# dylkot/cNMF

Hardware: AMD Instinct MI355X
Metric: NMF restarts/sec (50000x2000xK5..13) (higher is better)
Workload: dtype f32 (exact integer f16 plane x 2 f16 planes with per-row exponent, f32 accumulate)

## Files before the change

cnmf_amd/csrc/batch_host.hip.h:

```cpp
#pragma once

static int sweep_max_parts()
{
    static const int v = getenv("CNMF_SWEEP_PARTS") ? atoi(getenv("CNMF_SWEEP_PARTS")) : 64;
    return std::max(1, v);
}
static int sweep_chunks(int L) { const int64_t m = 256ll * sweep_max_parts(); return std::max(1, (int)(((int64_t)L + m - 1) / m)); }
static int sweep_parts(int L) { const int c = sweep_chunks(L); return (L + 256 * c - 1) / (256 * c); }

static int pick_nsplit(const cnmf_ctx* ctx, int KC)
{
    if (const char* s = ctx_getenv(ctx, "CNMF_NSPLIT")) { int v = atoi(s); if (v > 0) return v; }
    const int jt = (ctx->G_pad + 127) / 128;
    const int mg = std::max(1, KC / 128);
    int s = std::max(1, 512 / (jt * mg));
    const int max_by_k = std::max(1, ctx->N_pad / 256);
    return std::min(s, max_by_k);
}

static int effective_splits(int Ktot, int nsplit)
{
    const int Kper = round_up((Ktot + nsplit - 1) / nsplit, BK);
    return (Ktot + Kper - 1) / Kper;
}
// ... 212 lines not shown
        total_k += kk[r]; max_k = std::max(max_k, (int)kk[r]); min_k = std::min(min_k, (int)kk[r]);
        hoff[r + 1] = hoff[r] + (size_t)kk[r] * G;
        woff[r + 1] = woff[r] + (size_t)kk[r] * N;
    }
    const bool wide_can = gemm3_mode() != 0 && gemm3_enabled(ctx, 512);
    const char* ws_ = ctx_getenv(ctx, "CNMF_WIDE_SMALL");
    const bool wide_small = total_k >= 512 && !(ws_ && atoi(ws_) == 0);
    const bool wide_auto = wide_can && ((int64_t)ctx->N_pad * ctx->G_pad >= (1ll << 24) || wide_small);
    int KC = pick_kc(ctx, total_k, max_k, prm->kc_max, (prm->kc_max > 256 || ctx_getenv(ctx, "CNMF_KC")) ? wide_can : wide_auto);
    if (KC == 128 && prm->kc_max <= 0 && !ctx_getenv(ctx, "CNMF_KC") && gemm3_mode() >= 3 && gemm3_enabled(ctx, 256) &&
        (int64_t)ctx->N_pad * ctx->G_pad >= (1ll << 24)) {
        rc = ensure_counts(ctx);
        if (rc) return rc;
        if (ctx->count_state == 1) KC = 256;
    }
    const int KC0 = KC;
    rc = ensure_batch(ctx, KC, max_k, min_k);
    if (rc) return rc;
    rc = ensure_stage(ctx, (size_t)N * KMAX, (size_t)G * KMAX);
    if (rc) return rc;
    int nsplit = std::min(pick_nsplit(ctx, KC), ctx->nsplit_alloc);
    bool use3 = gemm3_enabled(ctx, KC);
    bool usec = false;
    if (use3 && gemm3_mode() >= 3) {
        rc = ensure_counts(ctx);
        if (rc) return rc;
        usec = ctx->count_state == 1;
    }
    static const bool g2g_off = getenv("CNMF_G2G") && atoi(getenv("CNMF_G2G")) == 0;
    bool use2g = use3 && !usec && gemm3_mode() >= 4 && !g2g_off && ctx->G_pad % G3C_JW == 0 && ctx->N_pad % G3C_JW == 0;
    if (use2g) { rc = ensure_x2planes(ctx); if (rc) return rc; }
    bool use2h = (usec && ctx->count_fmt == 4) || use2g;
    const int gemm_mode_used = !use3 ? 0 : (use2g ? 5 : (usec ? (use2h ? 4 : 3) : std::min(gemm3_mode(), 2)));
    const int KbA = ctx->G_pad / 16, KbB = ctx->N_pad / 16;
    const unsigned char *xA = use2g ? ctx->X2h : ctx->C1, *xAhi = use2g ? ctx->X2m : ctx->C1h;
    const unsigned char *xB = use2g ? ctx->Xt2h : ctx->Ct1, *xBhi = use2g ? ctx->Xt2m : ctx->Ct1h;
    const unsigned int *xAfl = use2g ? ctx->onesA : ctx->hiA, *xBfl = use2g ? ctx->onesB : ctx->hiB;
    const float *csA = use2g ? ctx->x2sA : nullptr, *csB = use2g ? ctx->x2sB : nullptr;
    const double* dsc = use2g ? nullptr : ctx->d_scale;
    const int nsubA = use2h ? gemm2h_nsub(xAhi != nullptr, KbA) : 1, nsubB = use2h ? gemm2h_nsub(xBhi != nullptr, KbB) : 1;
    static const bool fuse_off = getenv("CNMF_FUSE_W") && atoi(getenv("CNMF_FUSE_W")) == 0;
    const bool fuseW = use2h && !fuse_off && max_k <= KSMALL && ctx->shiftW != nullptr;
    int shgen = 0;
    int* const shW[2] = {ctx->shiftW, ctx->shiftW ? ctx->shiftW + ctx->kc_alloc : nullptr};
    if (fuseW) HIP_TRY(ctx, hipMemsetAsync(ctx->shiftW, 0, (size_t)3 * ctx->kc_alloc * sizeof(int), ctx->stream));
    if (use3 && !usec && !use2g) { rc = ensure_planes(ctx); if (rc) return rc; }
    const int jwA = (usec || use2g) ? G3C_JW : G3_JW;
    int nsplit3 = use3 ? pick_nsplit3(ctx, KC, jwA) : 1;
    const int nsplit3_first = nsplit3;
    const int fin_y = (max_k * max_k + 255) / 256;
    const int lag_env = ctx_getenv(ctx, "CNMF_LAG") ? atoi(ctx_getenv(ctx, "CNMF_LAG")) : 0;
    const int lag = std::max(1, std::min(RING - 2, prm->lag > 0 ? prm->lag : (lag_env > 0 ? lag_env : 2)));
    hipStream_t st = ctx->stream;

    DevPool pool;
    EventPool events;
    float* d_Hres = nullptr; float* d_Wres = nullptr;
    if (resident) {
        if (ctx->spectra_rows && ctx->spectra_G != G) {
            SET_ERR(ctx, "the resident store holds spectra over %lld genes, this matrix has %d: cnmf_spectra_reset first",
                    (long long)ctx->spectra_G, G);
            return CNMF_ESTATE;
        }
        ctx->spectra_G = G;
        const size_t need = (ctx->spectra_rows + (size_t)total_k) * G;
        if (need > ctx->spectra_cap) {
            float* nb = nullptr;
            const size_t cap = std::max(need, ctx->spectra_cap * 2);
            HIP_TRY(ctx, hipMalloc(&nb, cap * sizeof(float)));
            hipError_t ce = hipSuccess;
            if (ctx->spectra_rows)
                ce = hipMemcpyAsync(nb, ctx->spectra, ctx->spectra_rows * G * sizeof(float), hipMemcpyDeviceToDevice, st);
            if (ce == hipSuccess) ce = hipStreamSynchronize(st);
            if (ce != hipSuccess) { hipFree(nb); HIP_TRY(ctx, ce); }
            hipFree(ctx->spectra);
            ctx->spectra = nb; ctx->spectra_cap = cap;
        }
        d_Hres = ctx->spectra + ctx->spectra_rows * G;
    } else {
        d_Hres = pool.get<float>(hoff[n]);
    }
    if (W_out) d_Wres = pool.get<float>(woff[n]);
    int* d_repack = pool.get<int>((size_t)3 * KC0);
    POOL_TRY(ctx, pool);
    struct PinnedInts { int* p = nullptr; ~PinnedInts() { if (p) hipHostFree(p); } } repack_host;
    HIP_TRY(ctx, hipHostMalloc(&repack_host.p, (size_t)RING * 3 * KC0 * sizeof(int)));
    int* h_repack = repack_host.p;

    float *d_H0 = nullptr, *d_Wt0 = nullptr;
    RngJob* d_jobs = nullptr;
    if (init_mode == 1) {
        d_H0 = pool.get<float>(hoff[n]);
        d_Wt0 = pool.get<float>(woff[n]);
        d_jobs = pool.get<RngJob>((size_t)n);
        POOL_TRY(ctx, pool);
        std::vector<RngJob> jobs(n);
        int rowoff = 0;
        for (int r = 0; r < n; ++r) {
            jobs[r] = RngJob{seeds[r], kk[r], rowoff, avg[r], (long long)kk[r] * ((long long)G + N)};
            rowoff += kk[r];
        }
        HIP_TRY(ctx, hipMemcpy(d_jobs, jobs.data(), (size_t)n * sizeof(RngJob), hipMemcpyHostToDevice));
        rng_kernel<1><<<n, 256, 0, st>>>(d_jobs, nullptr, d_H0, G, G, d_Wt0, N, N);
        HIP_TRY(ctx, hipGetLastError());
    }

    std::vector<int> order(n);
    const bool queue_by_rank = ctx_getenv(ctx, "CNMF_QUEUE") && !strcmp(ctx_getenv(ctx, "CNMF_QUEUE"), "rank");
    const bool have_prior = ctx->iter_hint.size() == (size_t)KMAX + 1;
    auto prior_of = [&](int k) { return have_prior ? ctx->iter_hint[k] : 0.0; };
    if (queue_by_rank) {
        for (int r = 0; r < n; ++r) order[r] = r;
        std::stable_sort(order.begin(), order.end(), [&](int a, int b) { return kk[a] > kk[b]; });
    } else {
        std::vector<std::vector<int>> by_k(KMAX + 1);
        for (int r = 0; r < n; ++r) by_k[kk[r]].push_back(r);
        size_t pos = 0;
        for (size_t j = 0; pos < (size_t)n; ++j)
            for (int k = KMAX; k >= 1; --k)
                if (j < by_k[k].size()) order[pos++] = by_k[k][j];
        if (have_prior)
            std::stable_sort(order.begin(), order.end(), [&](int a, int b) {
                const double ea = prior_of(kk[a]) > 0 ? prior_of(kk[a]) : 1e30, eb = prior_of(kk[b]) > 0 ? prior_of(kk[b]) : 1e30;
                return ea > eb;
            });
    }
    std::vector<int64_t> k_iters(KMAX + 1, 0), k_done(KMAX + 1, 0);
    std::vector<double> rank_expect(KMAX + 1, 1e30);
    static const bool holes_fill = !(getenv("CNMF_HOLES") && !strcmp(getenv("CNMF_HOLES"), "wait"));
    if (have_prior)
        for (int k = 1; k <= KMAX; ++k) if (prior_of(k) > 0) rank_expect[k] = prior_of(k);
    int last_resort_done = 0;
    size_t next = 0;
    int n_pending = n;

    ColAlloc cols(KC);
    std::vector<HostSlot> hs(KC0);
    int nslots = 0;
    int n_active = 0;
    int64_t it = 0;
    int snap_nslots[RING] = {0};
    const bool no_defrag = ctx_getenv(ctx, "CNMF_NO_DEFRAG") != nullptr;
    const bool no_psum = ctx_getenv(ctx, "CNMF_NO_PSUM") != nullptr;
    const bool no_part = ctx_getenv(ctx, "CNMF_PART") == nullptr || ctx_getenv(ctx, "CNMF_NO_PART") != nullptr;
    int64_t last_tail_repack = -1000;
    int64_t last_defrag = -8, n_defrag = 0;
    bool h3_valid = false;
    memset(ctx->h_snap, 0, (size_t)ctx->kc_alloc * RING * sizeof(SlotDesc));
    hipEvent_t ev_begin = events.get(), ev_end = events.get();
    POOL_TRY(ctx, events);
    HIP_TRY(ctx, hipEventRecord(ev_begin, st));
    const int time_stride = !stats ? 0 : (prm->profile > 0 ? prm->profile : (ctx_getenv(ctx, "CNMF_TIME_GEMM") ? 1 : 0));
    std::vector<hipEvent_t> gev;

    const int chunksW = sweep_chunks(N), partsW = sweep_parts(N);
    const int chunksH = sweep_chunks(G), partsH = sweep_parts(G);
    const float l1W = (float)prm->l1_reg_W, l2W = (float)prm->l2_reg_W;
    const float l1H = (float)prm->l1_reg_H, l2H = (float)prm->l2_reg_H;
    const int gvarA = ctx_getenv(ctx, "CNMF_GEMM_A") ? atoi(ctx_getenv(ctx, "CNMF_GEMM_A")) : 0;
    const int gvarB = ctx_getenv(ctx, "CNMF_GEMM_B") ? atoi(ctx_getenv(ctx, "CNMF_GEMM_B")) : 0;
    int64_t restart_iters = 0, column_iters = 0, restart_col_iters = 0;
    const bool dbg = ctx_getenv(ctx, "CNMF_DEBUG") != nullptr;
    int64_t dbg_it[65] = {0}, dbg_live[65] = {0};
    const int wg_slots = ctx_getenv(ctx, "CNMF_SK_WGS") ? atoi(ctx_getenv(ctx, "CNMF_SK_WGS")) : 2 * 256;
    StreamK sk = plan_streamk(KC, ctx->N_pad, ctx->G_pad, wg_slots);
    if (sk.on) HIP_TRY(ctx, hipMemcpyAsync(ctx->d_split, sk.split.data(), sk.split.size(), hipMemcpyHostToDevice, st));
    int nsplitA = (sk.on && gvarA == 0) ? 1 : std::min(pick_nsplit_A(ctx, KC), ctx->nsplitA_alloc);
    StreamK3 sk3;
    if (use3) {
        sk3 = plan_streamk3(KC, ctx->N_pad, ctx->G_pad, gemm3_wg_slots(), jwA, nsubA);
        if (sk3.on) HIP_TRY(ctx, hipMemcpyAsync(ctx->d_split, sk3.flags.data(), sk3.flags.size(), hipMemcpyHostToDevice, st));
        else nsplitA = std::min(pick_nsplit_A3(ctx, KC, jwA), ctx->nsplitA_alloc);
    }
    int n_done = 0;
    hipEvent_t ev_tail = nullptr;
    int64_t tail_its = 0, tail_live = 0;

    auto retire = [&](int s, const SlotDesc& snap) -> int {
        HostSlot& h = hs[s];
        const int r = h.restart, k = h.k;
        dim3 gH((G + 255) / 256, k), gW((N + 255) / 256, k);
        extract_kernel<<<gH, 256, 0, st>>>(ctx->H, ctx->G_pad, G, h.off, k, d_Hres + hoff[r], 0);
        if (d_Wres) extract_kernel<<<gW, 256, 0, st>>>(ctx->Wt, ctx->N_pad, N, h.off, k, d_Wres + woff[r], 1);
        clear_rows_kernel<<<gH, 256, 0, st>>>(ctx->H, ctx->G_pad, ctx->G_pad, h.off, k);
        clear_rows_kernel<<<gW, 256, 0, st>>>(ctx->Wt, ctx->N_pad, ctx->N_pad, h.off, k);
        HIP_TRY(ctx, hipGetLastError());
        if (n_iter_out) n_iter_out[r] = snap.iter;
        if (viol_out) viol_out[r] = snap.viol_last;
        restart_iters += snap.iter;
        restart_col_iters += (int64_t)snap.iter * k;
        k_iters[k] += snap.iter; k_done[k] += 1;
        if (n_pending > 0) cols.release(h.off, k);
        h.state = 0; h.restart = -1;
        --n_active; ++n_done;
        return CNMF_OK;
    };

    int n_repack = 0;
    auto repack_left = [&](int width, bool balanced = false) -> int {
        std::vector<int> idx;
        for (int s = 0; s < nslots; ++s) if (hs[s].state) idx.push_back(s);
        std::sort(idx.begin(), idx.end(), [&](int a, int b) { return hs[a].off < hs[b].off; });
        int* hm = h_repack + (size_t)(n_repack++ % RING) * 3 * KC0;
        int* d_colmap = d_repack, *d_ids = d_repack + KC0, *d_offs = d_repack + 2 * KC0;
        int pos = 0, nmove = 0;
        const int ngroups = width / 256;
        if (balanced && ngroups > 1) {
            for (int c = 0; c < width; ++c) hm[c] = -1;
            std::vector<int> fill(ngroups, 0), byk(idx);
            std::stable_sort(byk.begin(), byk.end(), [&](int a, int b) { return hs[a].k > hs[b].k; });
            bool ok = true;
            std::vector<int> newoff(nslots, -1);
            for (int s : byk) {
                int g = -1;
                for (int q = 0; q < ngroups; ++q) if (fill[q] + hs[s].k <= 256 && (g < 0 || fill[q] < fill[g])) g = q;
                if (g < 0) { ok = false; break; }
                newoff[s] = g * 256 + fill[g]; fill[g] += hs[s].k;
            }
            if (ok) {
                for (int s : idx) {
                    HostSlot& h = hs[s];
                    for (int c = 0; c < h.k; ++c) hm[newoff[s] + c] = h.off + c;
                    if (h.off != newoff[s]) { hm[KC0 + nmove] = s; hm[2 * KC0 + nmove] = newoff[s]; ++nmove; h.off = newoff[s]; }
                }
                pos = 0;
            } else balanced = false;
        } else balanced = false;
        if (!balanced) {
        for (int s : idx) {
            HostSlot& h = hs[s];
            for (int c = 0; c < h.k; ++c) hm[pos + c] = h.off + c;
            if (h.off != pos) { hm[KC0 + nmove] = s; hm[2 * KC0 + nmove] = pos; ++nmove; h.off = pos; }
            pos += h.k;
        }
        for (int c = pos; c < width; ++c) hm[c] = -1;
        }
        if (nmove || pos < width) {
            HIP_TRY(ctx, hipMemcpyAsync(d_colmap, hm, (size_t)width * sizeof(int), hipMemcpyHostToDevice, st));
            gather_rows_cm_kernel<<<dim3((ctx->N_pad / 4 + 255) / 256, width), 256, 0, st>>>(ctx->Wt, ctx->N_pad, d_colmap, ctx->XHt);
            gather_rows_cm_kernel<<<dim3((ctx->G_pad / 4 + 255) / 256, width), 256, 0, st>>>(ctx->H, ctx->G_pad, d_colmap, ctx->XtW);
            HIP_TRY(ctx, hipGetLastError());
            HIP_TRY(ctx, hipMemcpyAsync(ctx->Wt, ctx->XHt, (size_t)width * ctx->N_pad * sizeof(float), hipMemcpyDeviceToDevice, st));
            HIP_TRY(ctx, hipMemcpyAsync(ctx->H, ctx->XtW, (size_t)width * ctx->G_pad * sizeof(float), hipMemcpyDeviceToDevice, st));
            if (fuseW) {
                int* tmp = ctx->shiftW + 2 * ctx->kc_alloc;
                for (int g2 = 0; g2 < 2; ++g2) {
                    permute_ints_kernel<<<(width + 255) / 256, 256, 0, st>>>(shW[g2], d_colmap, tmp, width);
                    HIP_TRY(ctx, hipMemcpyAsync(shW[g2], tmp, (size_t)width * sizeof(int), hipMemcpyDeviceToDevice, st));
                }
                HIP_TRY(ctx, hipGetLastError());
            }
            if (nmove) {
                HIP_TRY(ctx, hipMemcpyAsync(d_ids, hm + KC0, (size_t)nmove * sizeof(int), hipMemcpyHostToDevice, st));
                HIP_TRY(ctx, hipMemcpyAsync(d_offs, hm + 2 * KC0, (size_t)nmove * sizeof(int), hipMemcpyHostToDevice, st));
                set_slot_offs_kernel<<<(nmove + 255) / 256, 256, 0, st>>>(ctx->d_slots, d_ids, d_offs, nmove);
                HIP_TRY(ctx, hipGetLastError());
            }
        }
        h3_valid = false;
        if (use2h) HIP_TRY(ctx, launch_rowmax_part(st, ctx->Wt, ctx->N_pad, N, KC, chunksW * 256, nullptr, partsW, ctx->rmaxW));
        return CNMF_OK;
    };

    auto refill = [&](int& n_new) -> int {
        n_new = 0;
        int* new_list = ctx->h_slot_list + (size_t)(it % RING) * KC0;
        for (int attempt = 0; attempt < 2; ++attempt) {
        int failed_k = 1 << 30;
        int head_k = 0; double head_expect = 0.0;
        for (size_t pi = next; pi < order.size() && n_pending > 0; ++pi) {
            const int r = order[pi];
            if (r < 0) { if (pi == next) ++next; continue; }
            const int k = kk[r];
            if (k >= failed_k) continue;
            if (head_k && !holes_fill && !(rank_expect[k] < 0.3 * head_expect)) continue;
            const int off = cols.alloc(k);
            if (off < 0) {
                failed_k = k;
                if (!head_k) { head_k = k; head_expect = rank_expect[k]; }
                continue;
            }
            order[pi] = -1; --n_pending;
            if (pi == next) ++next;
            int s = 0;
            while (s < KC0 && hs[s].state != 0) ++s;
            hs[s].state = 1; hs[s].restart = r; hs[s].off = off; hs[s].k = k; hs[s].installed_at = it;
            nslots = std::max(nslots, s + 1);
            dim3 gI((std::max(N, G) + 255) / 256, k);
            if (init_mode == 0) {
                HIP_TRY(ctx, hipMemcpyAsync(ctx->stageH, H0 + hoff[r], (size_t)k * G * sizeof(float), hipMemcpyHostToDevice, st));
                HIP_TRY(ctx, hipMemcpyAsync(ctx->stageW, W0 + woff[r], (size_t)k * N * sizeof(float), hipMemcpyHostToDevice, st));
                install_kernel<<<gI, 256, 0, st>>>(ctx->stageH, ctx->stageW, ctx->H, ctx->G_pad, G, ctx->Wt, ctx->N_pad, N, off, k);
            } else {
                install_cm_kernel<<<gI, 256, 0, st>>>(d_H0 + hoff[r], d_Wt0 + woff[r], ctx->H, ctx->G_pad, G, ctx->Wt, ctx->N_pad, N, off);
            }
            HIP_TRY(ctx, hipGetLastError());
            if (fuseW) {
                float mx = 0.f;
                if (init_mode == 1) mx = 6.0f * (float)avg[r];
                else for (size_t q = 0; q < (size_t)k * N; ++q) mx = std::max(mx, W0[woff[r] + q]);
                int e2 = 0;
                if (mx > 0.f) std::frexp(mx, &e2);
                const int sh0 = mx > 0.f ? std::max(-110, std::min(120, 13 - e2)) : 0;
                set_ints_kernel<<<1, 128, 0, st>>>(shW[0], shW[1], off, k, sh0);
                HIP_TRY(ctx, hipGetLastError());
            }
            SlotDesc* d = &ctx->h_slots[s];
            memset(d, 0, sizeof *d);
            d->off = off; d->k = k; d->active = 1; d->iter = 0; d->restart = r;
            HIP_TRY(ctx, hipMemcpyAsync(ctx->d_slots + s, d, sizeof(SlotDesc), hipMemcpyHostToDevice, st));
            new_list[n_new++] = s;
            ++n_active;
        }
        if (attempt == 0 && n_pending > 0 && failed_k < (1 << 30) && !no_defrag && it - last_defrag >= 8) {
            int live_cols = 0;
            for (int s2 = 0; s2 < nslots; ++s2) if (hs[s2].state) live_cols += hs[s2].k;
            if (KC - live_cols >= (holes_fill ? failed_k : head_k)) {
                int rcd = repack_left(KC);
                if (rcd) return rcd;
                cols = ColAlloc(KC);
                for (int s2 = 0; s2 < nslots; ++s2) if (hs[s2].state) cols.alloc(hs[s2].k);
                last_defrag = it; ++n_defrag;
                continue;
            }
        }
        break;
        }
        if (n_new) {
            int* dl = ctx->d_slot_list + (size_t)(it % RING) * KC0;
            HIP_TRY(ctx, hipMemcpyAsync(dl, new_list, n_new * sizeof(int), hipMemcpyHostToDevice, st));
            gram_rows_kernel<<<n_new, 256, 0, st>>>(ctx->H, ctx->G_pad, G, ctx->d_slots, dl, ctx->gramH, l2W);
            HIP_TRY(ctx, hipGetLastError());
        }
        return CNMF_OK;
    };

    auto iterate = [&](int n_new) -> int {
        int tiers = 0;
        for (int s2 = 0; s2 < nslots; ++s2)
            if (hs[s2].state) tiers |= hs[s2].k <= 16 ? 1 : (hs[s2].k <= 32 ? 2 : (hs[s2].k <= KSMALL ? 4 : 8));
        unsigned long long livemask = ~0ull;
        if (use2h && n_pending == 0 && !no_part) {
            livemask = 0ull;
            for (int s2 = 0; s2 < nslots; ++s2)
                if (hs[s2].state)
                    for (int t = hs[s2].off / 32; t <= (hs[s2].off + hs[s2].k - 1) / 32 && t < 64; ++t) livemask |= 1ull << t;
            int fullest = 0;
            for (int g = 0; g < KC / 256; ++g) fullest = std::max(fullest, __builtin_popcountll((livemask >> (8 * g)) & 0xffull));
            if (fullest > 6) livemask = ~0ull;
        }
        const bool time_gemm = time_stride > 0 && it % time_stride == 0;
        if (time_gemm) {
            for (int i = 0; i < 4; ++i) gev.push_back(events.get());
            POOL_TRY(ctx, events);
            hipEventRecord(gev[gev.size() - 4], st);
        }
        SplitInfo spA{nullptr, nullptr, 1, 1, 1};
        if (use3) {
            if ((n_new > 0 || !h3_valid) && use2h) {
                HIP_TRY(ctx, launch_rowmax_part(st, ctx->H, ctx->G_pad, G, KC, chunksH * 256, dsc, partsH, ctx->rmaxH));
                HIP_TRY(ctx, launch_split2h(st, ctx->H, ctx->G_pad, KC, ctx->G_pad, ctx->H3, G3_MW, dsc, ctx->rmaxH,
                                            partsH, ctx->iscaleH));
            } else if (n_new > 0 || !h3_valid)
                HIP_TRY(ctx, launch_split3(st, ctx->H, ctx->G_pad, KC, ctx->G_pad, ctx->H3, G3_MW, usec ? ctx->d_scale : nullptr));
            if (time_gemm) hipEventRecord(gev[gev.size() - 4], st);
            if (sk3.on) {
                if (use2h) {
                    HIP_TRY(ctx, launch_gemm2h_streamk(st, sk3, ctx->H3, xA, xAhi, xAfl, ctx->iscaleH, KbA,
                                                       ctx->XHt, ctx->XHt1, ctx->XHt2, ctx->N_pad, csA, livemask));
                }
                else if (usec)
                    HIP_TRY(ctx, launch_gemm3c_streamk(st, sk3, ctx->H3, ctx->C1, ctx->C1h, ctx->hiA, ctx->XHt, ctx->XHt1,
                                                       ctx->XHt2, ctx->N_pad));
                else
                    HIP_TRY(ctx, launch_gemm3_streamk(st, sk3, ctx->H3, ctx->X3, ctx->XHt, ctx->XHt1, ctx->XHt2, ctx->N_pad));
                spA = SplitInfo{ctx->XHt1, ctx->d_split, jwA, G3_MW, sk3.MG, ctx->XHt2};
            } else if (use2h) {
                HIP_TRY(ctx, launch_gemm2h(st, ctx->H3, xA, xAhi, xAfl, ctx->iscaleH, KbA, ctx->XHt, ctx->N_pad,
                                           (long long)KC * ctx->N_pad, KC, ctx->N_pad, nsplitA, csA, livemask));
            } else if (usec) {
                HIP_TRY(ctx, launch_gemm3c(st, ctx->H3, ctx->C1, ctx->C1h, ctx->hiA, ctx->G_pad / 16, ctx->XHt, ctx->N_pad,
                                           (long long)KC * ctx->N_pad, KC, ctx->N_pad, nsplitA));
            } else {
                HIP_TRY(ctx, launch_gemm3(st, ctx->H3, ctx->X3, ctx->G_pad / 16, ctx->XHt, ctx->N_pad,
                                          (long long)KC * ctx->N_pad, KC, ctx->N_pad, nsplitA));
            }
        } else if (sk.on && gvarA == 0) {
            HIP_TRY(ctx, launch_streamk_passA(st, sk, ctx->H, ctx->G_pad, ctx->X, ctx->G_pad, ctx->XHt,
                                              ctx->XHt1, ctx->N_pad, ctx->N_pad));
            spA = SplitInfo{ctx->XHt1, ctx->d_split, 128, sk.mw, sk.MG};
        } else
            HIP_TRY(ctx, launch_gemm<false>(st, gvarA, ctx->H, ctx->G_pad, ctx->X, ctx->G_pad, ctx->XHt,
                                            ctx->N_pad, (long long)KC * ctx->N_pad, KC, ctx->G_pad, ctx->N_pad, nsplitA));
        if (time_gemm) hipEventRecord(gev[gev.size() - 3], st);
        if (!spA.plane1)
            HIP_TRY(ctx, launch_reduce_splits(st, ctx->XHt, use2h ? gemm2h_splits(KbA, nsplitA, nsubA) : nsplitA,
                                              (long long)KC * ctx->N_pad, (long long)KC * ctx->N_pad));
        const bool fuse_now = fuseW && use2h;
        HIP_TRY(ctx, launch_sweep(st, nslots, ctx->Wt, ctx->N_pad, N, ctx->XHt, ctx->gramH,
                                  ctx->d_slots, l1W, ctx->gram_part, ctx->viol_part, chunksW, partsW, 1, max_k, tiers, spA,
                                  use2h ? ctx->rmaxW : nullptr, nullptr, false,
                                  fuse_now ? PlaneOut{(unsigned short*)ctx->Wt3, shW[shgen], KbB, G3_MW} : PlaneOut{nullptr, nullptr, 0, 0}));
        if (use2h) {
            const FinalizeArgs fa{ctx->gram_part, ctx->viol_part, partsW, ctx->gramW, l2H, ctx->d_slots, 0, prm->tol,
                                  prm->max_iter, 1, max_k, nullptr, 0};
            HIP_TRY(ctx, launch_split2h_finalize(st, ctx->Wt, ctx->N_pad, KC, ctx->N_pad, ctx->Wt3, G3_MW, nullptr, ctx->rmaxW,
                                                 partsW, ctx->iscaleW, fa, nslots, fin_y,
                                                 fuse_now ? SplitFused{shW[shgen], shW[shgen ^ 1]} : SplitFused{nullptr, nullptr}));
            if (fuse_now) shgen ^= 1;
        } else if (use3) {
            const FinalizeArgs fa{ctx->gram_part, ctx->viol_part, partsW, ctx->gramW, l2H, ctx->d_slots, 0, prm->tol,
                                  prm->max_iter, 1, max_k, nullptr, 0};
            HIP_TRY(ctx, launch_split3_finalize(st, ctx->Wt, ctx->N_pad, KC, ctx->N_pad, ctx->Wt3, G3_MW, nullptr, fa,
                                                nslots, fin_y));
        } else {
            finalize_kernel<<<dim3(nslots, fin_y), 256, 0, st>>>(ctx->gram_part, ctx->viol_part, partsW, ctx->gramW, l2H,
                                                    ctx->d_slots, 0, prm->tol, prm->max_iter, 1, max_k);
        }
        if (time_gemm) hipEventRecord(gev[gev.size() - 2], st);
        const int nsB = use2h ? gemm2h_splits(KbB, nsplit3, nsubB) : (use3 ? nsplit3 : nsplit);
        if (use2h)
            HIP_TRY(ctx, launch_gemm2h(st, ctx->Wt3, xB, xBhi, xBfl, ctx->iscaleW, KbB, ctx->XtW, ctx->G_pad,
                                       (long long)KC * ctx->G_pad, KC, ctx->G_pad, nsplit3, csB, livemask));
        else if (usec)
            HIP_TRY(ctx, launch_gemm3c(st, ctx->Wt3, ctx->Ct1, ctx->Ct1h, ctx->hiB, ctx->N_pad / 16, ctx->XtW, ctx->G_pad,
                                       (long long)KC * ctx->G_pad, KC, ctx->G_pad, nsplit3));
        else if (use3)
            HIP_TRY(ctx, launch_gemm3(st, ctx->Wt3, ctx->Xt3, ctx->N_pad / 16, ctx->XtW, ctx->G_pad,
                                      (long long)KC * ctx->G_pad, KC, ctx->G_pad, nsplit3));
        else
            HIP_TRY(ctx, launch_gemm<true>(st, gvarB, ctx->Wt, ctx->N_pad, ctx->X, ctx->G_pad, ctx->XtW,
                                           ctx->G_pad, (long long)KC * ctx->G_pad, KC, ctx->N_pad,
                                           ctx->G_pad, nsplit));
        if (time_gemm) hipEventRecord(gev[gev.size() - 1], st);
        if (use2h && !no_psum && !(tiers & 8)) {
            HIP_TRY(ctx, launch_sweep(st, nslots, ctx->H, ctx->G_pad, G, ctx->XtW, ctx->gramW,
                                      ctx->d_slots, l1H, ctx->gram_part, ctx->viol_part, chunksH, partsH, 1, max_k, tiers,
                                      psum_info(nsB, (long long)KC * ctx->G_pad, dsc), ctx->rmaxH, dsc, true));
        } else {
            HIP_TRY(ctx, launch_reduce_splits(st, ctx->XtW, nsB, (long long)KC * ctx->G_pad,
                                              (long long)KC * ctx->G_pad, usec ? dsc : nullptr, ctx->G_pad));
            HIP_TRY(ctx, launch_sweep(st, nslots, ctx->H, ctx->G_pad, G, ctx->XtW, ctx->gramW,
                                      ctx->d_slots, l1H, ctx->gram_part, ctx->viol_part, chunksH, partsH, 1, max_k, tiers,
                                      SplitInfo{nullptr, nullptr, 1, 1, 1}, use2h ? ctx->rmaxH : nullptr,
                                      use2h ? dsc : nullptr));
        }
        SlotDesc* snap = ctx->h_snap + (size_t)(it % RING) * KC0;
        SlotDesc* snap_dev = nullptr;
        HIP_TRY(ctx, hipHostGetDevicePointer((void**)&snap_dev, snap, 0));
        if (use2h) {
            const FinalizeArgs fa{ctx->gram_part, ctx->viol_part, partsH, ctx->gramH, l2W, ctx->d_slots, 1, prm->tol,
                                  prm->max_iter, 1, max_k, snap_dev, (int)(it + 1)};
            HIP_TRY(ctx, launch_split2h_finalize(st, ctx->H, ctx->G_pad, KC, ctx->G_pad, ctx->H3, G3_MW, dsc,
                                                 ctx->rmaxH, partsH, ctx->iscaleH, fa, nslots, fin_y));
            h3_valid = true;
        } else if (use3) {
            const FinalizeArgs fa{ctx->gram_part, ctx->viol_part, partsH, ctx->gramH, l2W, ctx->d_slots, 1, prm->tol,
                                  prm->max_iter, 1, max_k, snap_dev, (int)(it + 1)};
            HIP_TRY(ctx, launch_split3_finalize(st, ctx->H, ctx->G_pad, KC, ctx->G_pad, ctx->H3, G3_MW,
                                                usec ? ctx->d_scale : nullptr, fa, nslots, fin_y));
            h3_valid = true;
        } else {
            finalize_kernel<<<dim3(nslots, fin_y), 256, 0, st>>>(ctx->gram_part, ctx->viol_part, partsH, ctx->gramH, l2W,
                                                    ctx->d_slots, 1, prm->tol, prm->max_iter, 1, max_k,
                                                    snap_dev, (int)(it + 1));
        }
        HIP_TRY(ctx, hipGetLastError());
        snap_nslots[it % RING] = nslots;
        column_iters += KC;
        if (n_pending == 0) {
            int live = 0;
            for (int s2 = 0; s2 < nslots; ++s2) if (hs[s2].state) live += hs[s2].k;
            ++tail_its; tail_live += live;
        }
        if (dbg) {
            int live = 0;
            for (int s2 = 0; s2 < nslots; ++s2) if (hs[s2].state) live += hs[s2].k;
            dbg_it[KC / 32] += 1; dbg_live[KC / 32] += live;
        }
        ++it;
        return CNMF_OK;
    };

    auto inspect = [&]() -> int {
        const int64_t si = it - 1 - lag;
        if (si < 0) return CNMF_OK;
        const SlotDesc* sp = ctx->h_snap + (size_t)(si % RING) * KC0;
        int rc2 = wait_snapshot(ctx, sp, snap_nslots[si % RING], (int)(si + 1));
        if (rc2) return rc2;
        for (int s = 0; s < snap_nslots[si % RING]; ++s)
            if (hs[s].state == 1 && hs[s].installed_at <= si && sp[s].active == 0 && sp[s].restart == hs[s].restart) {
                rc2 = retire(s, sp[s]);
                if (rc2) return rc2;
            }
        if (!queue_by_rank && n_pending > 1 && n_done - last_resort_done >= 8) {
            last_resort_done = n_done;
            std::vector<int> rest;
            rest.reserve(n_pending);
            for (size_t pi = next; pi < order.size(); ++pi) if (order[pi] >= 0) rest.push_back(order[pi]);
            std::vector<double> fly_age(KMAX + 1, 0.0); std::vector<int> fly_n(KMAX + 1, 0);
            for (int s2 = 0; s2 < nslots; ++s2)
                if (hs[s2].state) { fly_age[hs[s2].k] += (double)(it - hs[s2].installed_at); fly_n[hs[s2].k] += 1; }
            auto expect = [&](int r) {
                const int k = kk[r];
                double num = (double)k_iters[k] + fly_age[k], den = (double)k_done[k] + fly_n[k];
                if (prior_of(k) > 0) { num += 4.0 * prior_of(k); den += 4.0; }
                return den > 0 ? num / den : 1e30;
            };
            for (int k = 1; k <= KMAX; ++k) {
                const double den = (double)k_done[k] + fly_n[k] + (prior_of(k) > 0 ? 4.0 : 0.0);
                if (den > 0) rank_expect[k] = ((double)k_iters[k] + fly_age[k] + 4.0 * prior_of(k)) / den;
            }
            if (dbg && n_done % 64 < 8) {
                fprintf(stderr, "[cnmf] it %lld done %d pending %d expected per rank:", (long long)it, n_done, n_pending);
                for (int k = 1; k <= KMAX; ++k)
                    if (k_done[k] + fly_n[k] > 0)
                        fprintf(stderr, " k%d=%.0f(%lld done, %d fly)", k, ((double)k_iters[k] + fly_age[k]) / ((double)k_done[k] + fly_n[k]),
                                (long long)k_done[k], fly_n[k]);
                fprintf(stderr, "\n");
            }
            std::stable_sort(rest.begin(), rest.end(), [&](int a, int b) {
                const double ea = expect(a), eb = expect(b);
                return ea != eb ? ea > eb : kk[a] > kk[b];
            });
            order.resize(next);
            order.insert(order.end(), rest.begin(), rest.end());
        }
        return CNMF_OK;
    };

    const bool no_compact = ctx_getenv(ctx, "CNMF_NO_COMPACT") != nullptr;
    const bool f32_tail = ctx_getenv(ctx, "CNMF_F32_TAIL") != nullptr;
    auto compact = [&]() -> int {
        if (n_pending == 0 && n_active > 0 && KC > 32 && !no_compact) {
            int live_cols = 0;
            for (int s = 0; s < nslots; ++s) if (hs[s].state) live_cols += hs[s].k;
            int KCn = 32;
            while (KCn < live_cols && KCn < 256) KCn *= 2;
            if (live_cols > 256) KCn = round_up(live_cols, 256);
            bool stay3 = false;
            if (use3 && !f32_tail && KCn > (usec ? 32 : 64)) { KCn = round_up(std::max(live_cols, 1), 256); stay3 = true; }
            if (KCn == KC && use2h && !no_part && it - last_tail_repack >= 16) {
                unsigned long long m = 0ull;
                for (int s = 0; s < nslots; ++s)
                    if (hs[s].state)
                        for (int t = hs[s].off / 32; t <= (hs[s].off + hs[s].k - 1) / 32 && t < 64; ++t) m |= 1ull << t;
                const int ng = KC / 256;
                int fullest = 0;
                for (int g = 0; g < ng; ++g) fullest = std::max(fullest, __builtin_popcountll((m >> (8 * g)) & 0xffull));
                const int ideal = ((live_cols + 31) / 32 + ng - 1) / ng;
                if (ideal <= 6 && fullest >= ideal + 2) {
                    int rcp = repack_left(KC, true);
                    if (rcp) return rcp;
                    last_tail_repack = it;
                }
            }
            if (KCn < KC) {
                last_tail_repack = it;
                int rcp = repack_left(KCn, stay3 && use2h && !no_part);
                if (rcp) return rcp;
                KC = KCn;
                cols = ColAlloc(KC);
                for (int s = 0; s < nslots; ++s) if (hs[s].state) cols.alloc(hs[s].k);
                const int cap = (ctx->nsplit_alloc * KC0) / KC;
                if (stay3) {
                    nsplit3 = std::max(1, std::min(pick_nsplit3(ctx, KC, jwA), cap));
                    sk3 = plan_streamk3(KC, ctx->N_pad, ctx->G_pad, gemm3_wg_slots(), jwA, nsubA);
                    if (sk3.on) HIP_TRY(ctx, hipMemcpyAsync(ctx->d_split, sk3.flags.data(), sk3.flags.size(), hipMemcpyHostToDevice, st));
                    else nsplitA = std::max(1, std::min(pick_nsplit_A3(ctx, KC, jwA), (ctx->nsplitA_alloc * KC0) / KC));
                } else {
                nsplit = std::max(1, std::min(pick_nsplit(ctx, KC), cap));
                use3 = usec = use2h = use2g = false;
                sk = plan_streamk(KC, ctx->N_pad, ctx->G_pad, wg_slots);
                nsplitA = (sk.on && gvarA == 0) ? 1
                        : std::max(1, std::min(pick_nsplit_A(ctx, KC), (ctx->nsplitA_alloc * KC0) / KC));
                if (sk.on) {
                    HIP_TRY(ctx, hipMemcpyAsync(ctx->d_split, sk.split.data(), sk.split.size(), hipMemcpyHostToDevice, st));
// ... 167 lines not shown
```

cnmf_amd/csrc/cnmf_hip.hip:

```cpp
#include <hip/hip_runtime.h>

#include <algorithm>
#include <chrono>
#include <cmath>
#include <cstdint>
#include <cstdio>
#include <cstdlib>
#include <cstring>
#include <functional>
#include <string>
#include <vector>

#include "../../include/cnmf_hip.h"
#ifdef CNMF_DEBUG_ABI
#include "../../include/cnmf_hip_debug.h"
#endif
#include "kernels_gemm.hip.h"
#include "kernels_gemm3.hip.h"
#include "kernels_counts.hip.h"
#include "kernels_gemm2h.hip.h"
#include "kernels_rng.hip.h"
#include "kernels_sweep.hip.h"

using namespace cnmf;

#include "runtime.hip.h"
#include "csr_host.hip.h"
#include "gemm_host.hip.h"

extern "C" int cnmf_device_count(void)
{
    int n = 0;
    if (hipGetDeviceCount(&n) != hipSuccess) return 0;
    return n;
}

extern "C" const char* cnmf_version(void) { return "cnmf_hip 0.1.0 (gfx950)"; }

extern "C" const char* cnmf_last_error(const cnmf_ctx* ctx)
{
    return ctx ? ctx->err.c_str() : g_last_error.c_str();
}

extern "C" cnmf_ctx* cnmf_create(int device)
{
    int n = 0;
    hipError_t e = hipGetDeviceCount(&n);
    if (e != hipSuccess || n <= 0) {
        SET_ERR((cnmf_ctx*)nullptr, "no HIP device available (%s)", hipGetErrorString(e));
        return nullptr;
    }
    if (device < 0 || device >= n) {
        SET_ERR((cnmf_ctx*)nullptr, "device %d out of range (have %d)", device, n);
        return nullptr;
    }
    if (hipSetDevice(device) != hipSuccess) {
        SET_ERR((cnmf_ctx*)nullptr, "hipSetDevice(%d) failed", device);
        return nullptr;
    }
    cnmf_ctx* ctx = new cnmf_ctx();
    ctx_snapshot_env(ctx);
    ctx->device = device;
    if (hipStreamCreateWithFlags(&ctx->stream, hipStreamNonBlocking) != hipSuccess) {
        SET_ERR((cnmf_ctx*)nullptr, "hipStreamCreate failed");
        delete ctx;
        return nullptr;
    }
    return ctx;
}

extern "C" int cnmf_reload_env(cnmf_ctx* ctx)
{
    if (!ctx) return CNMF_EINVAL;
    ctx_snapshot_env(ctx);
    return CNMF_OK;
}

static void free_x2(cnmf_ctx* c)
{
    hipFree(c->X2h); hipFree(c->X2m); hipFree(c->Xt2h); hipFree(c->Xt2m); hipFree(c->x2sA); hipFree(c->x2sB);
    hipFree(c->onesA); hipFree(c->onesB);
    c->X2h = c->X2m = c->Xt2h = c->Xt2m = nullptr; c->x2sA = c->x2sB = nullptr; c->onesA = c->onesB = nullptr;
}

static void free_mu_sparse(cnmf_ctx* c)
{
    for (int i = 0; i < 2; ++i) { c->spA[i].release(); c->spB[i].release(); }
    c->x_nnz = -1;
}

static void free_batch(cnmf_ctx* c)
{
    hipFree(c->H); hipFree(c->Wt); hipFree(c->XHt); hipFree(c->XHt1); hipFree(c->XHt2); hipFree(c->XtW); hipFree(c->d_split);
    hipFree(c->H3); hipFree(c->Wt3);
    hipFree(c->rmaxH); hipFree(c->rmaxW); hipFree(c->iscaleH); hipFree(c->iscaleW); hipFree(c->shiftW);
    c->rmaxH = c->rmaxW = c->iscaleH = c->iscaleW = nullptr; c->shiftW = nullptr;
    c->XHt1 = c->XHt2 = nullptr; c->d_split = nullptr; c->H3 = c->Wt3 = nullptr;
    hipFree(c->gramH); hipFree(c->gramW); hipFree(c->gram_part); hipFree(c->viol_part);
    hipFree(c->d_slots); hipFree(c->d_slot_list);
    if (c->h_slots) hipHostFree(c->h_slots);
    if (c->h_snap) hipHostFree(c->h_snap);
    if (c->h_slot_list) hipHostFree(c->h_slot_list);
    c->H = c->Wt = c->XHt = c->XtW = c->gramH = c->gramW = c->gram_part = nullptr;
    c->viol_part = nullptr; c->d_slots = nullptr; c->d_slot_list = nullptr;
    c->h_slots = c->h_snap = nullptr; c->h_slot_list = nullptr;
// ... 192 lines not shown
```

Before: 221.6.

## Batch slot install and retire into event tables with fused kernels

Replaces the per-restart sequence of extract, clear, install, set_ints, SlotDesc memcpy and gram_rows launches with batched event tables. Each table is uploaded in one memcpy and processed by one fused retire kernel, or by an install kernel plus a gram-finish kernel. The Gram matrix of the initial H is now computed from the source buffer as chunked partials reduced in double. This cuts launch and small-copy overhead per restart. In exchange it adds pinned and device event buffers and a gram partial workspace, whose capacity limit forces extra flushes.

```diff
diff --git a/cnmf_amd/csrc/batch_host.hip.h b/cnmf_amd/csrc/batch_host.hip.h
--- a/cnmf_amd/csrc/batch_host.hip.h
+++ b/cnmf_amd/csrc/batch_host.hip.h
@@ -318,10 +318,19 @@
     }
     if (W_out) d_Wres = pool.get<float>(woff[n]);
     int* d_repack = pool.get<int>((size_t)3 * KC0);
+    const size_t evt_region = (size_t)KC0 * (sizeof(SlotRow) + sizeof(int) + 8);
+    unsigned char* d_evt = pool.get<unsigned char>(evt_region);
+    const int gram0_gc = max_k <= KSMALL ? 128 : 64;
+    const size_t gram0_per_slot = (size_t)((G + gram0_gc - 1) / gram0_gc) * max_k * max_k;
+    const int gram0_cap = (int)std::max<size_t>(1, std::min<size_t>((size_t)KC0 / min_k + 1, ((size_t)8 << 20) / gram0_per_slot));
+    float* d_gram0 = pool.get<float>((size_t)gram0_cap * gram0_per_slot);
     POOL_TRY(ctx, pool);
     struct PinnedInts { int* p = nullptr; ~PinnedInts() { if (p) hipHostFree(p); } } repack_host;
     HIP_TRY(ctx, hipHostMalloc(&repack_host.p, (size_t)RING * 3 * KC0 * sizeof(int)));
     int* h_repack = repack_host.p;
+    struct PinnedBytes { unsigned char* p = nullptr; ~PinnedBytes() { if (p) hipHostFree(p); } } evt_host;
+    HIP_TRY(ctx, hipHostMalloc(&evt_host.p, (size_t)RING * 2 * evt_region));
+    unsigned char* h_evt = evt_host.p;
 
     float *d_H0 = nullptr, *d_Wt0 = nullptr;
     RngJob* d_jobs = nullptr;
@@ -412,15 +421,68 @@
     hipEvent_t ev_tail = nullptr;
     int64_t tail_its = 0, tail_live = 0;
 
+    struct SlotEvent {
+        int64_t epoch = -1;
+        size_t used = 0;
+        SlotRow* rows = nullptr;
+        int nrows = 0, max_k = 0, stage_rows = 0;
+        std::vector<int> heads;
+    } ev_ret, ev_ins;
+    auto event_add = [&](SlotEvent& e, int kind, int s, long long hpos, long long wpos, int sh0) -> int {
+        const HostSlot& h = hs[s];
+        if (e.nrows == 0) {
+            if (e.epoch != it) { e.epoch = it; e.used = 0; }
+            e.rows = reinterpret_cast<SlotRow*>(h_evt + ((size_t)(it % RING) * 2 + kind) * evt_region + e.used);
+            e.max_k = 0; e.heads.clear();
+        }
+        if (e.used + (size_t)(e.nrows + h.k) * sizeof(SlotRow) + (e.heads.size() + 1) * sizeof(int) > evt_region) {
+            SET_ERR(ctx, "slot event table overflow (%d rows)", e.nrows + h.k);
+            return CNMF_ESTATE;
+        }
+        e.heads.push_back(e.nrows);
+        for (int c = 0; c < h.k; ++c) e.rows[e.nrows++] = SlotRow{h.off + c, h.k, c, s, hpos, wpos, sh0, h.restart, {0, 0}};
+        e.max_k = std::max(e.max_k, h.k);
+        return CNMF_OK;
+    };
+    auto event_upload = [&](SlotEvent& e) -> int {
+        memcpy(e.rows + e.nrows, e.heads.data(), e.heads.size() * sizeof(int));
+        const size_t bytes = (size_t)e.nrows * sizeof(SlotRow) + e.heads.size() * sizeof(int);
+        HIP_TRY(ctx, hipMemcpyAsync(d_evt, e.rows, bytes, hipMemcpyHostToDevice, st));
+        e.used += (bytes + 7) & ~(size_t)7;
+        return CNMF_OK;
+    };
+    auto flush_retire = [&]() -> int {
+        if (ev_ret.nrows == 0) return CNMF_OK;
+        if (int rcu = event_upload(ev_ret)) return rcu;
+        dim3 grid((std::max(ctx->G_pad, ctx->N_pad) + SLOT_CHUNK - 1) / SLOT_CHUNK, ev_ret.nrows);
+        slots_retire_kernel<<<grid, 256, 0, st>>>(reinterpret_cast<const SlotRow*>(d_evt), ctx->H, ctx->G_pad, G,
+                                                 ctx->Wt, ctx->N_pad, N, d_Hres, d_Wres);
+        HIP_TRY(ctx, hipGetLastError());
+        ev_ret.nrows = 0;
+        return CNMF_OK;
+    };
+    auto flush_install = [&]() -> int {
+        if (ev_ins.nrows == 0) return CNMF_OK;
+        if (int rcu = event_upload(ev_ins)) return rcu;
+        const SlotRow* d_rows = reinterpret_cast<const SlotRow*>(d_evt);
+        const int* d_heads = reinterpret_cast<const int*>(d_rows + ev_ins.nrows);
+        const int nsl = (int)ev_ins.heads.size(), gc = ev_ins.max_k <= KSMALL ? 128 : 64;
+        const int nch = (G + gc - 1) / gc, kk = ev_ins.max_k * ev_ins.max_k;
+        const int xch = (std::max(N, G) + SLOT_CHUNK - 1) / SLOT_CHUNK;
+        slots_install_kernel<<<xch * ev_ins.nrows + nch * nsl, 256, 0, st>>>(
+            d_rows, d_heads, ev_ins.nrows, xch, init_mode == 0 ? ctx->stageH : d_H0, init_mode == 0 ? ctx->stageW : d_Wt0,
+            init_mode == 0 ? 1 : 0, ctx->H, ctx->G_pad, G, ctx->Wt, ctx->N_pad, N, fuseW ? shW[0] : nullptr,
+            fuseW ? shW[1] : nullptr, ctx->d_slots, d_gram0, nch, kk);
+        slots_gram_finish_kernel<<<nsl, 256, 0, st>>>(d_rows, d_heads, d_gram0, nch, kk, G, ctx->gramH, l2W);
+        HIP_TRY(ctx, hipGetLastError());
+        ev_ins.nrows = 0; ev_ins.stage_rows = 0;
+        return CNMF_OK;
+    };
+
     auto retire = [&](int s, const SlotDesc& snap) -> int {
         HostSlot& h = hs[s];
         const int r = h.restart, k = h.k;
-        dim3 gH((G + 255) / 256, k), gW((N + 255) / 256, k);
-        extract_kernel<<<gH, 256, 0, st>>>(ctx->H, ctx->G_pad, G, h.off, k, d_Hres + hoff[r], 0);
-        if (d_Wres) extract_kernel<<<gW, 256, 0, st>>>(ctx->Wt, ctx->N_pad, N, h.off, k, d_Wres + woff[r], 1);
-        clear_rows_kernel<<<gH, 256, 0, st>>>(ctx->H, ctx->G_pad, ctx->G_pad, h.off, k);
-        clear_rows_kernel<<<gW, 256, 0, st>>>(ctx->Wt, ctx->N_pad, ctx->N_pad, h.off, k);
-        HIP_TRY(ctx, hipGetLastError());
+        if (int rce = event_add(ev_ret, 0, s, (long long)hoff[r], (long long)woff[r], 0)) return rce;
         if (n_iter_out) n_iter_out[r] = snap.iter;
         if (viol_out) viol_out[r] = snap.viol_last;
         restart_iters += snap.iter;
@@ -500,7 +562,6 @@
 
     auto refill = [&](int& n_new) -> int {
         n_new = 0;
-        int* new_list = ctx->h_slot_list + (size_t)(it % RING) * KC0;
         for (int attempt = 0; attempt < 2; ++attempt) {
         int failed_k = 1 << 30;
         int head_k = 0; double head_expect = 0.0;
@@ -522,36 +583,33 @@
             while (s < KC0 && hs[s].state != 0) ++s;
             hs[s].state = 1; hs[s].restart = r; hs[s].off = off; hs[s].k = k; hs[s].installed_at = it;
             nslots = std::max(nslots, s + 1);
-            dim3 gI((std::max(N, G) + 255) / 256, k);
+            if (ev_ins.nrows && ((int)ev_ins.heads.size() >= gram0_cap || (init_mode == 0 && ev_ins.stage_rows + k > KMAX)))
+                if (int rcf = flush_install()) return rcf;
+            long long hpos = (long long)hoff[r], wpos = (long long)woff[r];
             if (init_mode == 0) {
-                HIP_TRY(ctx, hipMemcpyAsync(ctx->stageH, H0 + hoff[r], (size_t)k * G * sizeof(float), hipMemcpyHostToDevice, st));
-                HIP_TRY(ctx, hipMemcpyAsync(ctx->stageW, W0 + woff[r], (size_t)k * N * sizeof(float), hipMemcpyHostToDevice, st));
-                install_kernel<<<gI, 256, 0, st>>>(ctx->stageH, ctx->stageW, ctx->H, ctx->G_pad, G, ctx->Wt, ctx->N_pad, N, off, k);
-            } else {
-                install_cm_kernel<<<gI, 256, 0, st>>>(d_H0 + hoff[r], d_Wt0 + woff[r], ctx->H, ctx->G_pad, G, ctx->Wt, ctx->N_pad, N, off);
-            }
-            HIP_TRY(ctx, hipGetLastError());
+                hpos = (long long)ev_ins.stage_rows * G; wpos = (long long)ev_ins.stage_rows * N;
+                HIP_TRY(ctx, hipMemcpyAsync(ctx->stageH + hpos, H0 + hoff[r], (size_t)k * G * sizeof(float), hipMemcpyHostToDevice, st));
+                HIP_TRY(ctx, hipMemcpyAsync(ctx->stageW + wpos, W0 + woff[r], (size_t)k * N * sizeof(float), hipMemcpyHostToDevice, st));
+                ev_ins.stage_rows += k;
+            }
+            int sh0 = 0;
             if (fuseW) {
                 float mx = 0.f;
                 if (init_mode == 1) mx = 6.0f * (float)avg[r];
                 else for (size_t q = 0; q < (size_t)k * N; ++q) mx = std::max(mx, W0[woff[r] + q]);
                 int e2 = 0;
                 if (mx > 0.f) std::frexp(mx, &e2);
-                const int sh0 = mx > 0.f ? std::max(-110, std::min(120, 13 - e2)) : 0;
-                set_ints_kernel<<<1, 128, 0, st>>>(shW[0], shW[1], off, k, sh0);
-                HIP_TRY(ctx, hipGetLastError());
-            }
-            SlotDesc* d = &ctx->h_slots[s];
-            memset(d, 0, sizeof *d);
-            d->off = off; d->k = k; d->active = 1; d->iter = 0; d->restart = r;
-            HIP_TRY(ctx, hipMemcpyAsync(ctx->d_slots + s, d, sizeof(SlotDesc), hipMemcpyHostToDevice, st));
-            new_list[n_new++] = s;
+                sh0 = mx > 0.f ? std::max(-110, std::min(120, 13 - e2)) : 0;
+            }
+            if (int rce = event_add(ev_ins, 1, s, hpos, wpos, sh0)) return rce;
+            ++n_new;
             ++n_active;
         }
         if (attempt == 0 && n_pending > 0 && failed_k < (1 << 30) && !no_defrag && it - last_defrag >= 8) {
             int live_cols = 0;
             for (int s2 = 0; s2 < nslots; ++s2) if (hs[s2].state) live_cols += hs[s2].k;
             if (KC - live_cols >= (holes_fill ? failed_k : head_k)) {
+                if (int rcf = flush_install()) return rcf;
                 int rcd = repack_left(KC);
                 if (rcd) return rcd;
                 cols = ColAlloc(KC);
@@ -562,13 +620,7 @@
         }
         break;
         }
-        if (n_new) {
-            int* dl = ctx->d_slot_list + (size_t)(it % RING) * KC0;
-            HIP_TRY(ctx, hipMemcpyAsync(dl, new_list, n_new * sizeof(int), hipMemcpyHostToDevice, st));
-            gram_rows_kernel<<<n_new, 256, 0, st>>>(ctx->H, ctx->G_pad, G, ctx->d_slots, dl, ctx->gramH, l2W);
-            HIP_TRY(ctx, hipGetLastError());
-        }
-        return CNMF_OK;
+        return flush_install();
     };
 
     auto iterate = [&](int n_new) -> int {
@@ -729,6 +781,7 @@
                 rc2 = retire(s, sp[s]);
                 if (rc2) return rc2;
             }
+        if ((rc2 = flush_retire())) return rc2;
         if (!queue_by_rank && n_pending > 1 && n_done - last_resort_done >= 8) {
             last_resort_done = n_done;
             std::vector<int> rest;
diff --git a/cnmf_amd/csrc/cnmf_hip.hip b/cnmf_amd/csrc/cnmf_hip.hip
--- a/cnmf_amd/csrc/cnmf_hip.hip
+++ b/cnmf_amd/csrc/cnmf_hip.hip
@@ -21,6 +21,7 @@
 #include "kernels_gemm2h.hip.h"
 #include "kernels_rng.hip.h"
 #include "kernels_sweep.hip.h"
+#include "kernels_slots.hip.h"
 
 using namespace cnmf;
 
diff --git a/cnmf_amd/csrc/kernels_slots.hip.h b/cnmf_amd/csrc/kernels_slots.hip.h
--- /dev/null
+++ b/cnmf_amd/csrc/kernels_slots.hip.h
@@ -0,0 +1,133 @@
+#pragma once
+#include <hip/hip_runtime.h>
+#include "kernels_sweep.hip.h"
+
+namespace cnmf {
+
+struct SlotRow {
+    int row;
+    int k;
+    int c;
+    int slot;
+    long long hpos;
+    long long wpos;
+    int sh0;
+    int restart;
+    int pad_[2];
+};
+static_assert(sizeof(SlotRow) == 48, "SlotRow is copied as raw bytes");
+
+constexpr int SLOT_CHUNK = 1024;
+
+__global__ __launch_bounds__(256) void slots_retire_kernel(const SlotRow* __restrict__ rows,
+                                                           float* __restrict__ H, int ldh, int G,
+                                                           float* __restrict__ Wt, int ldw, int N,
+                                                           float* __restrict__ Hres, float* __restrict__ Wres)
+{
+    const SlotRow r = rows[blockIdx.y];
+    float* h = H + (size_t)r.row * ldh;
+    float* w = Wt + (size_t)r.row * ldw;
+    float* ho = Hres + r.hpos + (size_t)r.c * G;
+    float* wo = Wres ? Wres + r.wpos + r.c : nullptr;
+#pragma unroll
+    for (int j = 0; j < SLOT_CHUNK / 256; ++j) {
+        const int i = blockIdx.x * SLOT_CHUNK + j * 256 + threadIdx.x;
+        if (i < ldh) {
+            if (i < G) ho[i] = h[i];
+            h[i] = 0.f;
+        }
+        if (i < ldw) {
+            if (wo && i < N) wo[(size_t)i * r.k] = w[i];
+            w[i] = 0.f;
+        }
+    }
+}
+
+template <int GC>
+__device__ __forceinline__ void gram_chunk_body(const float* __restrict__ src, int ld, int L, int k, int g0,
+                                                float* __restrict__ part, float* lds)
+{
+    float (*tile)[GC + 1] = reinterpret_cast<float (*)[GC + 1]>(lds);
+    const int tid = threadIdx.x;
+    for (int e = tid; e < k * GC; e += 256) {
+        const int c = e / GC, g = e % GC;
+        tile[c][g] = (g0 + g < L) ? src[(size_t)c * ld + g0 + g] : 0.f;
+    }
+    __syncthreads();
+    for (int e = tid; e < k * k; e += 256) {
+        const int a = e / k, b = e % k;
+        float s = 0.f;
+        for (int g = 0; g < GC; ++g) s = fmaf(tile[a][g], tile[b][g], s);
+        part[e] = s;
+    }
+}
+
+__global__ __launch_bounds__(256) void slots_install_kernel(const SlotRow* __restrict__ rows, const int* __restrict__ heads,
+                                                            int nrows, int xch,
+                                                            const float* __restrict__ H0, const float* __restrict__ W0, int w_rowmajor,
+                                                            float* __restrict__ H, int ldh, int G,
+                                                            float* __restrict__ Wt, int ldw, int N,
+                                                            int* __restrict__ shA, int* __restrict__ shB,
+                                                            SlotDesc* __restrict__ slots,
+                                                            float* __restrict__ gram_part, int nch, int kk)
+{
+    __shared__ __attribute__((aligned(16))) float lds[KMAX * 65];
+    const int b = blockIdx.x;
+    if (b < xch * nrows) {
+        const SlotRow r = rows[b / xch];
+        const int xc = b % xch;
+        const float* hs = H0 + r.hpos + (size_t)r.c * G;
+        const float* ws = w_rowmajor ? W0 + r.wpos + r.c : W0 + r.wpos + (size_t)r.c * N;
+        const size_t wstep = w_rowmajor ? (size_t)r.k : 1;
+        float* h = H + (size_t)r.row * ldh;
+        float* w = Wt + (size_t)r.row * ldw;
+#pragma unroll
+        for (int j = 0; j < SLOT_CHUNK / 256; ++j) {
+            const int i = xc * SLOT_CHUNK + j * 256 + threadIdx.x;
+            if (i < G) h[i] = hs[i];
+            if (i < N) w[i] = ws[(size_t)i * wstep];
+        }
+        if (xc == 0 && threadIdx.x == 0) {
+            if (shA) { shA[r.row] = r.sh0; shB[r.row] = r.sh0; }
+            if (r.c == 0) {
+                SlotDesc d;
+                d.off = r.row; d.k = r.k; d.active = 1; d.iter = 0; d.restart = r.restart; d.pad_ = 0;
+                d.viol = 0.0; d.viol_init = 0.0; d.viol_last = 0.0;
+                slots[r.slot] = d;
+            }
+        }
+    } else {
+        const int gb = b - xch * nrows;
+        const int j = gb / nch, chunk = gb % nch;
+        const SlotRow r = rows[heads[j]];
+        const float* src = H0 + r.hpos;
+        float* part = gram_part + ((size_t)j * nch + chunk) * kk;
+        if (r.k <= KSMALL) {
+            if (chunk * 128 < G) gram_chunk_body<128>(src, G, G, r.k, chunk * 128, part, lds);
+        } else {
+            if (chunk * 64 < G) gram_chunk_body<64>(src, G, G, r.k, chunk * 64, part, lds);
+        }
+    }
+}
+
+__global__ __launch_bounds__(256) void slots_gram_finish_kernel(const SlotRow* __restrict__ rows, const int* __restrict__ heads,
+                                                                const float* __restrict__ gram_part, int nch, int kk, int G,
+                                                                float* __restrict__ gram_out, float l2_reg)
+{
+    const int j = blockIdx.x;
+    const SlotRow r = rows[heads[j]];
+    const int k = r.k;
+    const int gc = k <= KSMALL ? 128 : 64;
+    const int n = (G + gc - 1) / gc;
+    const float* part = gram_part + (size_t)j * nch * kk;
+    for (int e = threadIdx.x; e < k * k; e += 256) {
+        double acc = 0.0;
+        for (int c = 0; c < n; ++c) acc += (double)part[(size_t)c * kk + e];
+        const int a = e / k, b = e % k;
+        float s = (float)acc;
+        if (a == b) s += l2_reg;
+        gram_out[(size_t)r.slot * GRAM_SZ + a * GRAM_LD + b] = s;
+    }
+}
+
+}
```

Measured after the change: 222.7 (median of 6 runs). About the same (+0.5%).
